# stein7/nerf-navigation

Measured on AMD Instinct MI355X. Metric: ray-samples/sec, Stonehenge-class 800x800 novel-view render, higher is better.
Workload: dtype f16

## Files before the change

nerf-navigation_amd/csrc/render_fused.hip:

```cpp
#include <atomic>
#include "ngp_mlp.h"
#include "ngp_sh.h"
#include "ngp_field.h"
#include "ngp_march.h"
#include "ngp_camera.h"

__global__ void k_field_forward_lds(rf_params P, const float* __restrict__ xyzs, const float* __restrict__ dirs, uint32_t M,
                                    float* __restrict__ sigmas, void* __restrict__ rgbs, bool rgb_half);

static int rf_field_forward(const ngp_field_t* field_host, const float* xyzs, const float* dirs, uint32_t M, float* sigmas, void* rgbs, bool rgb_half, void* stream) {
    rf_params P;
    int rc = rf_fill_params("field_forward", field_host, P);
    if (rc != NGP_OK) return rc;
    if (M == 0) return NGP_OK;
    NGP_REQUIRE(xyzs && dirs && sigmas && rgbs, "field_forward: null pointer");
    const uint32_t npairs = (M + 31) >> 5;
    uint32_t blocks = ngp_div_up(npairs, RF_BLOCK / 64);
    if (blocks > 256 * RF_FIELD_WG_PER_CU) blocks = 256 * RF_FIELD_WG_PER_CU;
    hipLaunchKernelGGL(k_field_forward_lds, dim3(blocks), dim3(RF_BLOCK), 36 * 1024, (hipStream_t)stream, P, xyzs, dirs, M, sigmas, rgbs, rgb_half);
    NGP_CHECK_LAUNCH("field_forward");
    return NGP_OK;
}

extern "C" int ngp_field_forward(const ngp_field_t* field_host, const float* xyzs, const float* dirs, uint32_t M,
                                 float* sigmas, float* rgbs, void* stream) {
    return rf_field_forward(field_host, xyzs, dirs, M, sigmas, rgbs, false, stream);
}

extern "C" int ngp_field_forward_half(const ngp_field_t* field_host, const float* xyzs, const float* dirs, uint32_t M,
                                      float* sigmas, void* rgbs_half, void* stream) {
    return rf_field_forward(field_host, xyzs, dirs, M, sigmas, rgbs_half, true, stream);
}


#ifndef RV_S
#define RV_S 12
#endif
static_assert(RV_S >= 2, "RV_S must be at least 2: the one-sample-per-round frame kernel has been removed");
#ifndef RV_BANDS
#define RV_BANDS 32u
#endif
#ifndef RV_REFILL_MIN
#define RV_REFILL_MIN 64
#endif
#ifndef RV_SLAB_STEPS
#define RV_SLAB_STEPS 16
#endif
#ifndef RV_BLOCK_THREADS
#define RV_BLOCK_THREADS 512
#endif
#ifndef RV_BLOCKS_PER_CU
#define RV_BLOCKS_PER_CU 1
#endif
static constexpr uint32_t RV_BLOCK = RV_BLOCK_THREADS;
static constexpr int RV_WAVES_PER_SIMD = (RV_BLOCK_THREADS / 256) * RV_BLOCKS_PER_CU;
static constexpr int RV_WAVES = RV_BLOCK / 64;
static constexpr uint32_t RV_LDS_W = RV_NFRAG * 1024;
static constexpr uint32_t RV_LDS_SH = RV_WAVES * 64 * 32;
static constexpr uint32_t RV_LDS_LV = 4 * 96;

struct rf_frame {
    const float* rays_o; const float* rays_d; uint32_t N;
    ngp_camera cam;
    const ngp_camera* cams; uint32_t frame_rays;
    float aabb[6]; float min_near;
    const uint8_t* bitfield; uint32_t C, H;
    float dt_gamma; uint32_t max_steps;
    float bg[3];
    float* image; float* depth; float* weights_sum;
    uint32_t* stats; uint32_t* queue;
#ifdef RV_COUNTERS
    uint32_t* hist;
#endif
    const uint32_t* coarse;
    uint32_t coarse_words;
    uint32_t tile_w;
    uint32_t skip;
    const uint32_t* occ_ext;
    float occ_unit, occ_top;
    const uint32_t* tile_perm;
};

__global__ __launch_bounds__(256) void k_build_coarse(const uint8_t* __restrict__ bitfield, uint32_t n_blocks_total,
                                                      uint32_t* __restrict__ coarse, uint32_t blocks_per_level, uint32_t C, uint32_t* __restrict__ ext) {
    const uint32_t w = blockIdx.x * 256 + threadIdx.x;
    if (w * 32 >= n_blocks_total) return;
    const uint64_t* b64 = reinterpret_cast<const uint64_t*>(bitfield);
    uint32_t bits = 0;
    #pragma unroll 8
    for (uint32_t i = 0; i < 32; i++) {
        const uint32_t blk = w * 32 + i;
        if (blk < n_blocks_total && b64[blk] != 0ull) bits |= 1u << i;
    }
    coarse[w] = bits;
    if (ext && bits) {
        uint32_t nb = 1;
        while (nb * nb * nb < blocks_per_level) nb <<= 1;
        uint32_t lo[3] = {0xFFFFFFFFu, 0xFFFFFFFFu, 0xFFFFFFFFu}, hi[3] = {0u, 0u, 0u};
        const uint32_t words_per_level = blocks_per_level / 32u, level = w / words_per_level;
        ngp_occ_extent_word(bits, w - level * words_per_level, level, C, nb, lo, hi);
        #pragma unroll
        for (int k = 0; k < 3; k++) { atomicMax(ext + k, (1u << 20) - lo[k]); atomicMax(ext + 3 + k, hi[k]); }
    }
}

struct rv_ray { float ox, oy, oz, dx, dy, dz, rdx, rdy, rdz; };
struct rv_consts {
    float bound, rbound, dt_gamma, dt_min, dt_max, rH, H3, Hf, Cf, Hm1;
    const uint8_t* grid;
    __device__ __forceinline__ int mip(int e) const { return (int)fminf(Cf - 1.0f, fmaxf(0.0f, (float)e)); }
};
__device__ __forceinline__ float rv_uniform(float v) {
    return __builtin_bit_cast(float, __builtin_amdgcn_readfirstlane(__builtin_bit_cast(int, v)));
}
struct rv_view : rv_ray, rv_consts {
    __device__ __forceinline__ rv_view(const rv_ray& r, const rv_consts& k) : rv_ray(r), rv_consts(k) {}
};

typedef ngp_point<rv_view> rv_point;

struct rv_block_cache { uint32_t blk = 0xffffffffu, lo = 0, hi = 0; };

struct rv_tested { rv_point r; bool maybe; uint32_t sw; };

__device__ __forceinline__ bool rv_test(const rv_view& m, const uint32_t* __restrict__ lds_coarse, uint32_t coarse_words, rv_block_cache& bc,
                                        float tc, rv_tested& st
#ifdef RV_COUNTERS
                                        , int* rv_dbg_ptr
#endif
                                        ) {
    rv_point& r = st.r;
    r.at(m, tc);
    const uint32_t mort = ngp_morton3((uint32_t)r.nx, (uint32_t)r.ny, (uint32_t)r.nz);
    st.maybe = true;
    st.sw = 0;
    if (lds_coarse) {
        const uint32_t blk = mort >> 6;
        st.maybe = (lds_coarse[(uint32_t)r.level * coarse_words + (blk >> 5)] >> (blk & 31u)) & 1u;
        st.sw = (uint32_t)r.level * coarse_words + ((blk >> 6) << 1);
#ifdef RV_COUNTERS
        *rv_dbg_ptr = st.maybe ? 0 : ((lds_coarse[st.sw] | lds_coarse[st.sw + 1]) == 0u ? 2 : 1);
#endif
    }
    if (!st.maybe) return false;
    if (lds_coarse) {
        const uint32_t gblk = (uint32_t)r.level * (coarse_words << 5) + (mort >> 6);
        if (gblk != bc.blk) {
            const uint2 w = reinterpret_cast<const uint2*>(m.grid)[gblk];
            bc.blk = gblk; bc.lo = w.x; bc.hi = w.y;
        }
        return (((mort & 32u) ? bc.hi : bc.lo) >> (mort & 31u)) & 1u;
    }
    const uint32_t index = (uint32_t)((float)r.level * m.H3 + (float)mort);
    return (m.grid[index >> 3] >> (index & 7u)) & 1u;
}

__device__ __forceinline__ float rv_leave(const rv_view& m, const uint32_t* __restrict__ lds_coarse, float M, const rv_tested& st, float tc) {
    const rv_point& r = st.r;
    const float tt = r.cell_exit(m, tc);
    if (lds_coarse && !st.maybe) {
        const int sh = ((lds_coarse[st.sw] | lds_coarse[st.sw + 1]) == 0u) ? 4 : 2;
        const float ta = ngp_try_skip(m, r, tc, tt, sh, M);
        if (ta >= 0.0f) return ta;
    }
    float tp;
    return ngp_advance(m, tc, tt, tp);
}

__device__ __forceinline__ bool rv_probe(const rv_ray& ray, const rv_consts& k, const uint32_t* __restrict__ lds_coarse, uint32_t coarse_words,
                                         float M, rv_block_cache& bc, float& t, float& x, float& y, float& z, float& dt
#ifdef RV_COUNTERS
                                         , int* rv_dbg_ptr
#endif
                                         ) {
    const rv_view m(ray, k);
    rv_tested st;
#ifdef RV_COUNTERS
    const bool occ = rv_test(m, lds_coarse, coarse_words, bc, t, st, rv_dbg_ptr);
#else
    const bool occ = rv_test(m, lds_coarse, coarse_words, bc, t, st);
#endif
    x = st.r.x; y = st.r.y; z = st.r.z; dt = st.r.dt;
    if (occ) return true;
    t = rv_leave(m, lds_coarse, M, st, t);
    return false;
}


template <bool FIXED>
__device__ __forceinline__ void rf_points_loop(const rf_params& P, const rf_iter_class cls_rt, const rf_lane_levels& lv, const ngp_h8* __restrict__ lds_w,
                                               const float* __restrict__ xyzs, const float* __restrict__ dirs, uint32_t M,
                                               float* __restrict__ sigmas, void* __restrict__ rgbs_v, bool rgb_half) {
    const rf_iter_class cls = FIXED ? rf_iter_class{1u, 12u, 2u} : cls_rt;
    const int lane = threadIdx.x & 63, g = lane >> 4, s = lane & 15;
    const uint32_t wave = (blockIdx.x * RF_BLOCK + threadIdx.x) >> 6, nwaves = gridDim.x * (RF_BLOCK / 64);
    const uint32_t npairs = (M + 31) >> 5;
    for (uint32_t pair = wave; pair < npairs; pair += nwaves) {
        ngp_h8 x[2];
        ngp_h4 shq[2];
        uint32_t m[2];
        #pragma unroll
        for (int n = 0; n < 2; n++) {
            m[n] = pair * 32 + 16 * n + s;
            const uint64_t mm = m[n] < M ? m[n] : 0;
            const float px = xyzs[3 * mm], py = xyzs[3 * mm + 1], pz = xyzs[3 * mm + 2];
            float sh[16];
            sh_eval<4>(dirs[3 * mm], dirs[3 * mm + 1], dirs[3 * mm + 2], P.shn, sh);
            #pragma unroll
            for (int j = 0; j < 4; j++) {
                float v = sh[j];
                if (g == 1) v = sh[4 + j];
                if (g == 2) v = sh[8 + j];
                if (g == 3) v = sh[12 + j];
                shq[n][j] = ngp_f2h(v);
            }
            x[n] = rf_encode<false>(P, lv, cls, px, py, pz);
        }
        float sg[2], cr[2], cg[2], cb[2];
        rv_mlp_tiles<2>(lds_w, lane, x, shq, sg, cr, cg, cb);
        #pragma unroll
        for (int n = 0; n < 2; n++)
            if (g == 0 && m[n] < M) {
                rv_activate(P, sg[n], cr[n], cg[n], cb[n]);
                sigmas[m[n]] = sg[n];
                if (rgb_half) {
                    _Float16* rgbs = static_cast<_Float16*>(rgbs_v);
                    rgbs[3ull * m[n]] = (_Float16)cr[n]; rgbs[3ull * m[n] + 1] = (_Float16)cg[n]; rgbs[3ull * m[n] + 2] = (_Float16)cb[n];
                } else {
                    float* rgbs = static_cast<float*>(rgbs_v);
                    rgbs[3ull * m[n]] = cr[n]; rgbs[3ull * m[n] + 1] = cg[n]; rgbs[3ull * m[n] + 2] = cb[n];
                }
            }
    }
}

__global__ __launch_bounds__(RF_BLOCK, RF_FIELD_WG_PER_CU) void k_field_forward_lds(rf_params P, const float* __restrict__ xyzs, const float* __restrict__ dirs,
                                                                    uint32_t M, float* __restrict__ sigmas, void* __restrict__ rgbs, bool rgb_half) {
    extern __shared__ __attribute__((aligned(16))) unsigned char rf_smem[];
    ngp_h8* lds_w = reinterpret_cast<ngp_h8*>(rf_smem);
    const int lane = threadIdx.x & 63, g = lane >> 4, wave = threadIdx.x >> 6;
    rv_stage_weights(P, lds_w, wave, RF_BLOCK / 64, lane);
    rf_lane_levels lv;
    rf_setup_levels(P, g, lv);
    __syncthreads();
    const rf_iter_class cls = rf_classify(lv);
    if (cls.dense == 1u && cls.select == 2u && cls.hashed == 12u) rf_points_loop<true>(P, cls, lv, lds_w, xyzs, dirs, M, sigmas, rgbs, rgb_half);
    else rf_points_loop<false>(P, cls, lv, lds_w, xyzs, dirs, M, sigmas, rgbs, rgb_half);
}

__device__ __forceinline__ void rv_ray_od(const rf_frame& F, uint32_t ray, float o[3], float d[3]) {
    if (F.rays_o) {
        #pragma unroll
        for (int k = 0; k < 3; k++) { o[k] = F.rays_o[3ull * ray + k]; d[k] = F.rays_d[3ull * ray + k]; }
    } else if (F.cams) {
        const uint32_t f = ray / F.frame_rays;
        const ngp_camera c = F.cams[f];
        o[0] = c.t[0]; o[1] = c.t[1]; o[2] = c.t[2];
        ngp_camera_ray(c, ray - f * F.frame_rays, d);
    } else {
        o[0] = F.cam.t[0]; o[1] = F.cam.t[1]; o[2] = F.cam.t[2];
        ngp_camera_ray(F.cam, ray, d);
    }
}

__device__ __forceinline__ uint32_t rv_ray_of(uint32_t idx, uint32_t tile_w) {
    if (tile_w == 0) return idx;
    const uint32_t tile = idx >> 6, in = idx & 63u, tiles_x = tile_w >> 3;
    const uint32_t ty = tile / tiles_x, tx = tile - ty * tiles_x;
    const uint32_t p = in >> 4, s = in & 15u;
    const uint32_t px = (p & 1u) * 4 + (s & 3u), py = (p >> 1) * 4 + (s >> 2);
    return (ty * 8 + py) * tile_w + tx * 8 + px;
}

static constexpr uint32_t RV_LDS_SMP = RV_WAVES * 64 * RV_S * 16;

template <bool FIXED>
__device__ __forceinline__ void rv_frame_loop(const rf_params& P, const rf_frame& F, const rf_iter_class cls_rt,
                                              const ngp_h8* __restrict__ lds_w, _Float16* lds_sh, const rf_lane_levels* lds_lv,
                                              float4* lds_smp, const uint32_t* lds_coarse, const float* lds_occ) {
    const rf_iter_class cls = FIXED ? rf_iter_class{1u, 12u, 2u} : cls_rt;
    const int lane = threadIdx.x & 63, g = lane >> 4, s = lane & 15, wave = threadIdx.x >> 6;
    const int wave_s = __builtin_amdgcn_readfirstlane(wave);

    _Float16* my_sh = lds_sh + (wave * 64 + lane) * 16;
    const _Float16* wave_sh = lds_sh + wave * 64 * 16;
    float4* my_smp = lds_smp + (wave * 64 + lane) * RV_S;
    float4* wave_smp = lds_smp + wave * 64 * RV_S;

    rv_consts K;
    K.bound = P.bound; K.rbound = rv_uniform(1.0f / P.bound); K.dt_gamma = F.dt_gamma;
    K.Hf = rv_uniform((float)F.H); K.Cf = rv_uniform((float)F.C); K.Hm1 = rv_uniform((float)(F.H - 1));
    K.rH = rv_uniform(1.0f / K.Hf);
    K.H3 = rv_uniform((float)(F.H * F.H * F.H));
    K.dt_min = rv_uniform((2.0f * 1.7320508075688772f) / (float)F.max_steps);
    K.dt_max = rv_uniform(((2.0f * 1.7320508075688772f) * (float)(1 << (F.C - 1))) / K.Hf);
    K.grid = F.bitfield;

    bool active = false;
    uint32_t ray = 0, nsamp = 0;
    rv_ray m;
    float t = 0, last_t = 0, near = 0, far = 0;
    float ws = 0, dacc = 0, cr = 0, cg = 0, cb = 0, tcomp = 0;
    bool exhausted = false;
    uint32_t rv_q = blockIdx.x & 7u, rv_q_seen = 0;
    rv_block_cache bc;
    uint32_t n_samples_local = 0, n_tiles = 0, n_capped_local = 0, n_hit_local = 0;
#ifdef RV_COUNTERS
    uint32_t n_rounds = 0, n_trips = 0, n_probe[4] = {0, 0, 0, 0};
    unsigned long long c_refill = 0, c_march = 0, c_tiles = 0, c_comp = 0;
    const unsigned long long c_start = __builtin_readcyclecounter();
    unsigned long long c_last = c_start;
#define RV_TICK(acc) { const unsigned long long c_now = __builtin_readcyclecounter(); acc += c_now - c_last; c_last = c_now; }
    uint32_t* rv_hist = F.hist;
    unsigned long long rv_t0 = 0;
    if (rv_hist) {
        unsigned long long* p0 = reinterpret_cast<unsigned long long*>(F.queue + 24);
        const unsigned long long now = wall_clock64();
        const unsigned long long old = atomicCAS(p0, 0ull, now);
        rv_t0 = __shfl(old ? old : now, 0, 64);
    }
#else
#define RV_TICK(acc)
#endif

    for (;;) {
        if (!exhausted) {
            const unsigned long long need = __ballot(!active);
            if (need && (uint32_t)__popcll(need) >= RV_REFILL_MIN) {
                const uint32_t cnt = (uint32_t)__popcll(need);
                uint32_t base = 0;
                const uint32_t n_tiles64 = (F.N + 63u) >> 6;
                const uint32_t q_lo = (uint32_t)(((unsigned long long)n_tiles64 * rv_q) / RV_BANDS) << 6;
                uint32_t q_hi = (uint32_t)(((unsigned long long)n_tiles64 * (rv_q + 1u)) / RV_BANDS) << 6;
                q_hi = q_hi < F.N ? q_hi : F.N;
                if (lane == 0) base = atomicAdd(F.queue + 32 + rv_q, cnt);
                base = __shfl(base, 0, 64) + q_lo;
                if (!active) {
                    const uint32_t idx = base + (uint32_t)__popcll(need & ((1ull << lane) - 1ull));
                    if (idx < q_hi) {
                        ray = rv_ray_of(F.tile_perm ? (F.tile_perm[idx >> 6] << 6) | (idx & 63u) : idx, F.tile_w);
                        float o[3], d[3];
                        rv_ray_od(F, ray, o, d);
                        ngp_near_far_inline(o, d, F.aabb, F.min_near, near, far);
                        if (lds_occ) {
                            float n2, f2;
                            ngp_near_far_inline(o, d, lds_occ, 0.0f, n2, f2);
                            far = f2 == 3.402823466e+38f ? near : fminf(far, f2 + lds_occ[6]);
                        }
                        m.ox = o[0]; m.oy = o[1]; m.oz = o[2];
                        m.dx = d[0]; m.dy = d[1]; m.dz = d[2];
                        m.rdx = 1.0f / m.dx; m.rdy = 1.0f / m.dy; m.rdz = 1.0f / m.dz;
                        t = near; last_t = near; tcomp = near;
                        ws = 0; dacc = 0; cr = 0; cg = 0; cb = 0; nsamp = 0;
                        float sh[16];
                        sh_eval<4>(m.dx, m.dy, m.dz, P.shn, sh);
                        #pragma unroll
                        for (int j = 0; j < 16; j++) my_sh[j] = ngp_f2h(sh[j]);
                        active = true;
                    }
                }
                if (base + cnt >= q_hi) {
                    rv_q += 8u;
                    if (rv_q >= RV_BANDS) rv_q = (rv_q + 1u) & 7u;
                    if (++rv_q_seen == RV_BANDS) exhausted = true;
                }
            }
        }
        if (__ballot(active) == 0ull) {
            if (exhausted) break;
            continue;
        }
        RV_TICK(c_refill)

        int cnt = 0;
        bool ended = false;
#ifdef RV_COUNTERS
        n_rounds++;
        const unsigned long long rv_live = __ballot(active);
#endif
        {
            rv_ray mr = m;
            float far_r = far;
            asm("" : "+v"(mr.ox), "+v"(mr.oy), "+v"(mr.oz), "+v"(mr.dx), "+v"(mr.dy), "+v"(mr.dz),
                     "+v"(mr.rdx), "+v"(mr.rdy), "+v"(mr.rdz), "+v"(far_r));
            rv_consts Kr = K;
            asm("" : "+v"(Kr.Hf), "+v"(Kr.Hm1), "+v"(Kr.Cf), "+v"(Kr.rH), "+v"(Kr.dt_min), "+v"(Kr.dt_max), "+v"(Kr.rbound), "+v"(Kr.H3));
            const float M = (active && F.skip) ? ngp_skip_margin(mr, K.bound, lds_occ ? far_r + 4.0f * K.bound : far_r) : __builtin_inff();
            const uint32_t slot0 = ((uint32_t)wave_s * 64u + __builtin_amdgcn_mbcnt_hi(~0u, __builtin_amdgcn_mbcnt_lo(~0u, 0u))) * RV_S;
            float4* const smp_w = lds_smp + slot0;
            int probes = 0;
            float t_lim = __builtin_inff();
            auto march = [&](int upto) {
                for (;;) {
#ifdef RV_COUNTERS
                    n_trips = __builtin_amdgcn_readfirstlane(n_trips) + 1;
#endif
                    if (!(t < far_r && nsamp < F.max_steps)) { ended = true; break; }
                    if (RV_SLAB_STEPS > 0 && !(t < t_lim)) break;
                    float x, y, z, dt;
#ifdef RV_COUNTERS
                    int pc = 0;
                    const bool hit = rv_probe(mr, Kr, lds_coarse, F.coarse_words, M, bc, t, x, y, z, dt, &pc);
                    n_probe[pc]++;
                    if (hit) {
#else
                    if (rv_probe(mr, Kr, lds_coarse, F.coarse_words, M, bc, t, x, y, z, dt)) {
#endif
                        smp_w[cnt] = make_float4(x, y, z, t);
                        t += dt;
                        nsamp++;
                        if (++cnt >= upto) break;
                    }
                    if (++probes >= RF_PROBES_PER_ROUND) break;
                }
            };
            if (RV_SLAB_STEPS > 0) {
                if (active) march(1);
                const float t_first = cnt ? smp_w[0].w : __builtin_inff();
                float tf = t_first;
                #pragma unroll
                for (int off = 1; off < 64; off <<= 1) tf = fminf(tf, __shfl_xor(tf, off, 64));
                t_lim = tf + (float)RV_SLAB_STEPS * K.dt_min;
                if (cnt && !(t_first < t_lim)) { t = t_first; nsamp--; cnt = 0; ended = false; }
                if (active && cnt && !ended) march(RV_S);
            } else if (active) {
                march(RV_S);
            }
        }

        __builtin_amdgcn_fence(__ATOMIC_RELEASE, "wavefront");
        __builtin_amdgcn_wave_barrier();
        __builtin_amdgcn_fence(__ATOMIC_ACQUIRE, "wavefront");

        RV_TICK(c_march)
        int col_src;
        {
            uint32_t rank = 0, above = 0;
            const uint32_t below_me = __builtin_amdgcn_mbcnt_hi(~0u, __builtin_amdgcn_mbcnt_lo(~0u, 0u));
            #pragma unroll
            for (int c = RV_S; c >= 0; c--) {
                const unsigned long long mc = __ballot(cnt == c);
                if (cnt == c) rank = above + (uint32_t)__popcll(mc & ((1ull << below_me) - 1ull));
                above += (uint32_t)__popcll(mc);
            }
            col_src = __builtin_amdgcn_ds_permute((int)(rank << 2), (int)below_me);
        }
        #pragma unroll 1
        for (int p = 0; p < 4; p++) {
            const int src = __shfl(col_src, 16 * p + s, 64);
            const int ccol = __shfl(cnt, src, 64);
            if (__ballot(ccol > 0) == 0ull) continue;
            const ngp_h4 shq = *reinterpret_cast<const ngp_h4*>(wave_sh + src * 16 + 4 * g);
            const rf_lane_levels lv = lds_lv[g];
            #pragma unroll 1
            for (int k = 0; k < RV_S; k += 2) {
                if (__ballot(ccol > k) == 0ull) break;
                if (k + 1 < RV_S && __ballot(ccol > k + 1) != 0ull) {
                    ngp_h8 xs[2];
                    #pragma unroll
                    for (int n = 0; n < 2; n++) {
                        float4 q = wave_smp[src * RV_S + k + n];
                        if (!(ccol > k + n)) q = make_float4(0.f, 0.f, 0.f, 0.f);
                        xs[n] = rf_encode<true>(P, lv, cls, q.x, q.y, q.z);
                    }
                    n_tiles += 2;
                    const ngp_h4 ss[2] = {shq, shq};
                    float a[2], b[2], c[2], d[2];
                    rv_mlp_tiles<2>(lds_w, lane, xs, ss, a, b, c, d);
                    #pragma unroll
                    for (int n = 0; n < 2; n++)
                        if (g == 0 && ccol > k + n) {
                            ngp_h4 r;
                            r[0] = (_Float16)a[n]; r[1] = (_Float16)b[n]; r[2] = (_Float16)c[n]; r[3] = (_Float16)d[n];
                            *reinterpret_cast<ngp_h4*>(&wave_smp[src * RV_S + k + n]) = r;
                        }
                } else {
                    float4 q = wave_smp[src * RV_S + k];
                    if (!(ccol > k)) q = make_float4(0.f, 0.f, 0.f, 0.f);
                    n_tiles++;
                    float a, b, c, d;
                    rv_field_tile(P, lv, cls, lds_w, lane, q.x, q.y, q.z, shq, a, b, c, d);
                    if (g == 0 && ccol > k) {
                        ngp_h4 r;
                        r[0] = (_Float16)a; r[1] = (_Float16)b; r[2] = (_Float16)c; r[3] = (_Float16)d;
                        *reinterpret_cast<ngp_h4*>(&wave_smp[src * RV_S + k]) = r;
                    }
                }
            }
        }

        __builtin_amdgcn_fence(__ATOMIC_RELEASE, "wavefront");
        __builtin_amdgcn_wave_barrier();
        __builtin_amdgcn_fence(__ATOMIC_ACQUIRE, "wavefront");

        RV_TICK(c_tiles)
        bool done = false;
        for (int k = 0; k < cnt; k++) {
            const ngp_h4 r = *reinterpret_cast<const ngp_h4*>(&my_smp[k]);
            const float ts = my_smp[k].w;
            const float dt = ngp_clampf(ts * K.dt_gamma, K.dt_min, K.dt_max);
            const float ta = ts + dt;
            const float d1 = ta - last_t;
            last_t = ta;
            float sig = (float)r[0], sr = (float)r[1], sg = (float)r[2], sb = (float)r[3];
            rv_activate(P, sig, sr, sg, sb);
            n_samples_local++;
            const float alpha = 1.0f - ngp_expf(-sig * dt);
            const float T = 1 - ws;
            const float w = alpha * T;
            ws += w;
            tcomp += d1;
            dacc += w * tcomp;
            cr += w * sr; cg += w * sg; cb += w * sb;
            if ((double)T < 1e-4) {
                done = true;
#ifdef RV_COUNTERS
                n_probe[3] += (uint32_t)(cnt - (k + 1));
#endif
                break;
            }
        }
        float far0 = far;
        if (lds_occ && (done || ended)) {
            const float o3[3] = {m.ox, m.oy, m.oz}, d3[3] = {m.dx, m.dy, m.dz};
            float n0;
            ngp_near_far_inline(o3, d3, F.aabb, F.min_near, n0, far0);
        }
        const bool capped = !done && ended && nsamp >= F.max_steps && t < far0;
        if (ended) done = true;
        if (done) {
            F.image[3ull * ray] = cr + (1 - ws) * F.bg[0];
            F.image[3ull * ray + 1] = cg + (1 - ws) * F.bg[1];
            F.image[3ull * ray + 2] = cb + (1 - ws) * F.bg[2];
            F.depth[ray] = fmaxf(dacc - near, 0.0f) / (far0 - near);
            F.weights_sum[ray] = ws;
            n_capped_local += capped ? 1u : 0u;
            n_hit_local += nsamp > 0 ? 1u : 0u;
            active = false;
        }
        RV_TICK(c_comp)
#ifdef RV_COUNTERS
        if (rv_hist) {
            const unsigned long long now = wall_clock64();
            const uint32_t bin = now > rv_t0 ? (uint32_t)((now - rv_t0) / 2000ull) : 0u;
            uint32_t rs = (uint32_t)cnt;
            #pragma unroll
            for (int off = 32; off > 0; off >>= 1) rs += __shfl_down(rs, off, 64);
            if (lane == 0 && bin < 512u) {
                atomicAdd(rv_hist + bin, rs); atomicAdd(rv_hist + 512 + bin, 1u);
                atomicAdd(rv_hist + 1024 + bin, (uint32_t)__popcll(rv_live));
            }
        }
#endif
    }
#ifdef RV_COUNTERS
    if (rv_hist && lane == 0) {
        const unsigned long long now = wall_clock64();
        const uint32_t bin = now > rv_t0 ? (uint32_t)((now - rv_t0) / 2000ull) : 0u;
        if (bin < 512u) atomicAdd(rv_hist + 1536 + bin, 1u);
    }
#endif
    uint32_t tot = n_samples_local, tot_capped = n_capped_local, tot_hit = n_hit_local;
    #pragma unroll
    for (int off = 32; off > 0; off >>= 1) {
        tot += __shfl_down(tot, off, 64);
        tot_capped += __shfl_down(tot_capped, off, 64);
        tot_hit += __shfl_down(tot_hit, off, 64);
    }
    if (lane == 0 && tot) atomicAdd(F.stats, tot);
    if (lane == 0 && tot_capped) atomicAdd(F.stats + 1, tot_capped);
    if (lane == 0 && tot_hit) atomicAdd(F.stats + 2, tot_hit);
    if (lane == 0 && n_tiles) atomicAdd(F.stats + 3, n_tiles);
#ifdef RV_COUNTERS
    if (lane == 0) { atomicAdd(F.queue + 1, n_rounds); atomicAdd(F.queue + 2, n_trips); }
    atomicAdd(F.queue + 3, n_probe[0]); atomicAdd(F.queue + 4, n_probe[1]); atomicAdd(F.queue + 5, n_probe[2]); atomicAdd(F.queue + 6, n_probe[3]);
    if (lane == 0) {
        unsigned long long* c = reinterpret_cast<unsigned long long*>(F.queue + 8);
        const unsigned long long c_total = __builtin_readcyclecounter() - c_start;
        atomicAdd(c + 0, c_refill); atomicAdd(c + 1, c_march); atomicAdd(c + 2, c_tiles); atomicAdd(c + 3, c_comp);
        atomicAdd(c + 4, c_total); atomicMax(c + 5, c_total); atomicMax(c + 6, ~c_total);
    }
#endif
}

__global__ __launch_bounds__(RV_BLOCK, RV_WAVES_PER_SIMD) void k_render_frame_multi(rf_params P, rf_frame F) {
    extern __shared__ __attribute__((aligned(16))) unsigned char rv_smem[];
    ngp_h8* lds_w = reinterpret_cast<ngp_h8*>(rv_smem);
    _Float16* lds_sh = reinterpret_cast<_Float16*>(rv_smem + RV_LDS_W);
    rf_lane_levels* lds_lv = reinterpret_cast<rf_lane_levels*>(rv_smem + RV_LDS_W + RV_LDS_SH);
    float4* lds_smp = reinterpret_cast<float4*>(rv_smem + RV_LDS_W + RV_LDS_SH + RV_LDS_LV);
    uint32_t* lds_coarse = F.coarse ? reinterpret_cast<uint32_t*>(rv_smem + RV_LDS_W + RV_LDS_SH + RV_LDS_LV + RV_LDS_SMP) : nullptr;

    const int lane = threadIdx.x & 63, g = lane >> 4, s = lane & 15, wave = threadIdx.x >> 6;

    rv_stage_weights(P, lds_w, wave, RV_WAVES, lane);
    if (lds_coarse) {
        const uint32_t nw = F.coarse_words * F.C;
        for (uint32_t i = threadIdx.x; i < nw; i += RV_BLOCK) lds_coarse[i] = F.coarse[i];
    }
    float* lds_occ = (lds_coarse && F.occ_ext) ? reinterpret_cast<float*>(lds_coarse + F.coarse_words * F.C) : nullptr;
    if (lds_occ && threadIdx.x < 3) {
        const uint32_t k = threadIdx.x;
        const uint32_t hi = F.occ_ext[3 + k], lo = (1u << 20) - F.occ_ext[k];
        const bool any = F.occ_ext[3] != 0u;
        lds_occ[k] = any ? -F.occ_top + ((float)lo - 1.0f) * F.occ_unit : 3.0e38f;
        lds_occ[3 + k] = any ? -F.occ_top + ((float)hi + 1.0f) * F.occ_unit : 3.1e38f;
        if (k == 0) lds_occ[6] = 2.0f * (((2.0f * 1.7320508075688772f) * (float)(1 << (F.C - 1))) / (float)F.H);
    }
    if (wave == 0 && s == 0) {
        rf_lane_levels tmp;
        rf_setup_levels(P, g, tmp);
        lds_lv[g] = tmp;
    }
    __syncthreads();
    const rf_iter_class cls = rf_classify(lds_lv[g]);
    if (cls.dense == 1u && cls.select == 2u && cls.hashed == 12u)
        rv_frame_loop<true>(P, F, cls, lds_w, lds_sh, lds_lv, lds_smp, lds_coarse, lds_occ);
    else
        rv_frame_loop<false>(P, F, cls, lds_w, lds_sh, lds_lv, lds_smp, lds_coarse, lds_occ);
}

static constexpr uint32_t RV_ORDER_MAX = 4096;

__global__ __launch_bounds__(256) void k_tile_cost(rf_frame F, float bound, uint32_t n_tiles, uint32_t* __restrict__ cost) {
    const uint32_t tile = blockIdx.x * 4u + (threadIdx.x >> 6), lane = threadIdx.x & 63u;
    if (tile >= n_tiles) return;
    rv_consts K;
    K.bound = bound; K.rbound = 1.0f / bound; K.dt_gamma = F.dt_gamma;
    K.Hf = (float)F.H; K.Cf = (float)F.C; K.Hm1 = (float)(F.H - 1); K.rH = 1.0f / K.Hf; K.H3 = (float)(F.H * F.H * F.H);
    K.dt_min = (2.0f * 1.7320508075688772f) / (float)F.max_steps;
    K.dt_max = ((2.0f * 1.7320508075688772f) * (float)(1 << (F.C - 1))) / K.Hf;
    K.grid = F.bitfield;
    float box[7] = {0.f, 0.f, 0.f, 0.f, 0.f, 0.f, 0.f};
    if (F.occ_ext) {
        const bool any = F.occ_ext[3] != 0u;
        #pragma unroll
        for (int k = 0; k < 3; k++) {
            const uint32_t hi = F.occ_ext[3 + k], lo = (1u << 20) - F.occ_ext[k];
            box[k] = any ? -F.occ_top + ((float)lo - 1.0f) * F.occ_unit : 3.0e38f;
            box[3 + k] = any ? -F.occ_top + ((float)hi + 1.0f) * F.occ_unit : 3.1e38f;
        }
        box[6] = 2.0f * K.dt_max;
    }
    const uint32_t tiles_x = F.tile_w >> 3, ty = tile / tiles_x, tx = tile - ty * tiles_x;
    float acc = 0.0f;
    #pragma unroll
    for (int r = 0; r < 5; r++) {
        const uint32_t px = r == 4 ? 4u : (r & 1) * 7u, py = r == 4 ? 4u : (r >> 1) * 7u;
        float o[3], d[3], near, far;
        rv_ray_od(F, (ty * 8u + py) * F.tile_w + tx * 8u + px, o, d);
        ngp_near_far_inline(o, d, F.aabb, F.min_near, near, far);
        if (F.occ_ext) {
            float n2, f2;
            ngp_near_far_inline(o, d, box, 0.0f, n2, f2);
            far = f2 == 3.402823466e+38f ? near : fminf(far, f2 + box[6]);
        }
        rv_ray m;
        m.ox = o[0]; m.oy = o[1]; m.oz = o[2]; m.dx = d[0]; m.dy = d[1]; m.dz = d[2]; m.rdx = m.rdy = m.rdz = 0.0f;
        const rv_view v(m, K);
        const float seg = far > near ? (far - near) * (1.0f / 64.0f) : 0.0f;
        rv_point pt;
        pt.at(v, (far > near ? near : 0.0f) + ((float)lane + 0.5f) * seg);
        const uint32_t blk = ngp_morton3((uint32_t)pt.nx, (uint32_t)pt.ny, (uint32_t)pt.nz) >> 6;
        if ((F.coarse[(uint32_t)pt.level * F.coarse_words + (blk >> 5)] >> (blk & 31u)) & 1u) acc += seg / pt.dt;
    }
    #pragma unroll
    for (int off = 32; off > 0; off >>= 1) acc += __shfl_xor(acc, off, 64);
    if (lane == 0) cost[tile] = (uint32_t)fminf(acc + 0.5f, 4.0e9f);
}

__global__ __launch_bounds__(1024) void k_tile_sort(const uint32_t* __restrict__ cost, uint32_t n_tiles, uint32_t* __restrict__ perm) {
    __shared__ __attribute__((aligned(16))) uint32_t c[RV_ORDER_MAX];
    const uint32_t b = blockIdx.x;
    const uint32_t lo = (uint32_t)(((unsigned long long)n_tiles * b) / RV_BANDS), hi = (uint32_t)(((unsigned long long)n_tiles * (b + 1u)) / RV_BANDS);
    const uint32_t n = hi - lo, n4 = (n + 3u) & ~3u;
    for (uint32_t i = threadIdx.x; i < n4; i += 1024u) c[i] = i < n ? cost[lo + i] : 0u;
    __syncthreads();
    const uint4* c4 = reinterpret_cast<const uint4*>(c);
    for (uint32_t i = threadIdx.x; i < n; i += 1024u) {
        const uint32_t ci = c[i];
        uint32_t rank = 0;
        #pragma unroll 4
        for (uint32_t j = 0; j < n4; j += 4u) {
            const uint4 q = c4[j >> 2];
            rank += (q.x > ci || (q.x == ci && j < i)) ? 1u : 0u;
            rank += (q.y > ci || (q.y == ci && j + 1u < i)) ? 1u : 0u;
            rank += (q.z > ci || (q.z == ci && j + 2u < i)) ? 1u : 0u;
            rank += (q.w > ci || (q.w == ci && j + 3u < i)) ? 1u : 0u;
        }
        perm[lo + rank] = lo + i;
    }
}

static inline bool rv_pow2(uint32_t v) { return v && !(v & (v - 1)); }

static std::atomic<int> rv_occ_box_enabled{1};
extern "C" int ngp_render_set_occupied_box(int enabled) { return rv_occ_box_enabled.exchange(enabled ? 1 : 0, std::memory_order_relaxed); }
static std::atomic<int> rv_block_skip_enabled{1};
extern "C" int ngp_render_set_block_skip(int enabled) { return rv_block_skip_enabled.exchange(enabled ? 1 : 0, std::memory_order_relaxed); }
static std::atomic<int> rv_tile_order_enabled{1};
extern "C" int ngp_render_set_tile_order(int enabled) { return rv_tile_order_enabled.exchange(enabled ? 1 : 0, std::memory_order_relaxed); }

static constexpr size_t RV_WS_COARSE = 256, RV_WS_HIST = RV_WS_COARSE + 36 * 1024, RV_WS_AREA = 256 + 48 * 1024;
static_assert(RV_LDS_W + RV_LDS_SH + RV_LDS_LV + RV_LDS_SMP + 36 * 1024 > 160 * 1024, "the coarse map could reach RV_WS_HIST");
static_assert(RV_WS_HIST + 2048 * sizeof(uint32_t) <= RV_WS_AREA, "workspace carve");
extern "C" size_t ngp_render_frame_workspace(uint32_t N) {
    return RV_WS_AREA + 2 * sizeof(uint32_t) * (size_t)ngp_div_up(N, 64u);
}

static int rv_fill_camera(const char* who, const float* pose_host, const float* intrinsics_host, uint32_t H, uint32_t W, ngp_camera& cam) {
    NGP_REQUIRE(pose_host && intrinsics_host, "camera: pose / intrinsics are host pointers and must not be null");
    NGP_REQUIRE(H >= 1 && W >= 1 && (uint64_t)H * W <= 0xFFFFFFFFull, "camera: bad image size");
    NGP_REQUIRE(intrinsics_host[0] != 0.0f && intrinsics_host[1] != 0.0f, "camera: zero focal length");
    for (int r = 0; r < 3; r++) {
        for (int c = 0; c < 3; c++) cam.r[3 * r + c] = pose_host[4 * r + c];
        cam.t[r] = pose_host[4 * r + 3];
    }
    cam.fx = intrinsics_host[0]; cam.fy = intrinsics_host[1]; cam.cx = intrinsics_host[2]; cam.cy = intrinsics_host[3];
    cam.W = W; cam.H = H;
    (void)who;
    return NGP_OK;
}

static int rv_render_frame(const ngp_field_t* field_host, const float* rays_o, const float* rays_d, const ngp_camera* cam, uint32_t n_cams, uint32_t N,
                           uint32_t image_width, const float* aabb_host, float min_near, const uint8_t* bitfield, uint32_t C, uint32_t Hgrid,
                           float dt_gamma, uint32_t max_steps, const float* bg_color3_host,
                           float* image, float* depth, float* weights_sum, uint32_t* stats,
                           void* workspace, size_t workspace_bytes, void* stream) {
    rf_params P;
    int rc = rf_fill_params("render_frame", field_host, P);
    if (rc != NGP_OK) return rc;
    NGP_REQUIRE(stats && workspace && workspace_bytes >= RV_WS_COARSE, "render_frame: stats / workspace missing");
    NGP_REQUIRE(aabb_host && bg_color3_host, "render_frame: aabb / bg_color are host pointers and must not be null");
    NGP_REQUIRE(C >= 1 && C <= 16 && Hgrid >= 1 && Hgrid <= 1024 && max_steps >= 1, "render_frame: bad C/H/max_steps");
    NGP_REQUIRE(rv_pow2(Hgrid), "render_frame: the grid size must be a power of two (cells are addressed by Morton index)");
    hipStream_t s = (hipStream_t)stream;
    if (hipMemsetAsync(stats, 0, 4 * sizeof(uint32_t), s) != hipSuccess || hipMemsetAsync(workspace, 0, RV_WS_COARSE, s) != hipSuccess)
        return ngp_fail(NGP_ELAUNCH, "render_frame: memset failed");
    if (N == 0) return NGP_OK;
    NGP_REQUIRE((cam || (rays_o && rays_d)) && bitfield && image && depth && weights_sum, "render_frame: null pointer");
    rf_frame F;
    F.rays_o = cam ? nullptr : rays_o; F.rays_d = cam ? nullptr : rays_d; F.N = N;
    F.cam = cam ? *cam : ngp_camera{};
    F.cams = nullptr; F.frame_rays = N;
    if (cam && n_cams > 1) {
        const size_t at = (ngp_render_frame_workspace(N) + 255) & ~(size_t)255;
        NGP_REQUIRE(workspace_bytes >= at + n_cams * sizeof(ngp_camera), "render_frames_camera: workspace too small (ngp_render_frames_workspace)");
        ngp_camera* dst = reinterpret_cast<ngp_camera*>(reinterpret_cast<unsigned char*>(workspace) + at);
        if (hipMemcpyAsync(dst, cam, n_cams * sizeof(ngp_camera), hipMemcpyHostToDevice, s) != hipSuccess) return ngp_fail(NGP_ELAUNCH, "render_frames_camera: camera copy failed");
        F.cams = dst; F.frame_rays = N / n_cams;
    }
    for (int i = 0; i < 6; i++) F.aabb[i] = aabb_host[i];
    F.min_near = min_near; F.bitfield = bitfield; F.C = C; F.H = Hgrid;
    F.dt_gamma = dt_gamma; F.max_steps = max_steps;
    for (int i = 0; i < 3; i++) F.bg[i] = bg_color3_host[i];
    F.image = image; F.depth = depth; F.weights_sum = weights_sum;
    F.stats = stats; F.queue = (uint32_t*)workspace;
#ifdef RV_COUNTERS
    F.hist = nullptr;
#ifdef RV_TIMELINE
    if (workspace_bytes >= RV_WS_HIST + 2048 * sizeof(uint32_t)) {
        F.hist = reinterpret_cast<uint32_t*>(reinterpret_cast<unsigned char*>(workspace) + RV_WS_HIST);
        if (hipMemsetAsync(F.hist, 0, 2048 * sizeof(uint32_t), s) != hipSuccess) return ngp_fail(NGP_ELAUNCH, "render_frame: memset failed");
    }
#endif
#endif
    F.tile_w = 0;
    const uint32_t hint = image_width;
    if (hint >= 8 && hint % 8 == 0 && N % hint == 0 && (N / hint) % 8 == 0) F.tile_w = hint;

    F.coarse = nullptr; F.coarse_words = 0; F.skip = 0; F.occ_ext = nullptr; F.occ_unit = 0.0f; F.occ_top = 0.0f;
    F.tile_perm = nullptr;
    static_assert(sizeof(rf_lane_levels) * 4 == RV_LDS_LV, "LDS carve of the level table");
    size_t lds = RV_LDS_W + RV_LDS_SH + RV_LDS_LV + RV_LDS_SMP;
    const void* kernel = reinterpret_cast<const void*>(k_render_frame_multi);
    const uint64_t blocks_per_level = (uint64_t)Hgrid * Hgrid * Hgrid / 64;
    const uint64_t coarse_bytes = (uint64_t)C * blocks_per_level / 8;
    if (rv_pow2(Hgrid) && Hgrid >= 8 && blocks_per_level % 32 == 0 && lds + coarse_bytes <= 160 * 1024 && (uint64_t)C * Hgrid * Hgrid * Hgrid <= (1ull << 24) &&
        workspace_bytes >= RV_WS_COARSE + coarse_bytes && (reinterpret_cast<uintptr_t>(bitfield) & 7u) == 0) {
        uint32_t* coarse = reinterpret_cast<uint32_t*>(reinterpret_cast<unsigned char*>(workspace) + RV_WS_COARSE);
        const uint32_t n_blocks_total = (uint32_t)(C * blocks_per_level);
        F.coarse = coarse;
        F.coarse_words = (uint32_t)(blocks_per_level / 32);
        lds += coarse_bytes;
        uint32_t* ext = nullptr;
        int e2;
        const bool nested = Hgrid >= 64 && (C == 1 || frexpf(field_host->bound, &e2) == 0.5f);
        if (nested && rv_occ_box_enabled.load(std::memory_order_relaxed) && lds + 32 <= 160 * 1024) {
            ext = reinterpret_cast<uint32_t*>(workspace) + 26;
            F.occ_ext = ext;
            F.occ_top = C == 1 ? field_host->bound : (float)(1u << (C - 1));
            F.occ_unit = 2.0f * (C == 1 ? field_host->bound : 1.0f) / (float)(Hgrid / 4);
            lds += 32;
        }
        hipLaunchKernelGGL(k_build_coarse, dim3(ngp_div_up(n_blocks_total / 32, 256)), dim3(256), 0, s, bitfield, n_blocks_total, coarse,
                           (uint32_t)blocks_per_level, C, ext);
        int e;
        F.skip = (rv_block_skip_enabled.load(std::memory_order_relaxed) && Hgrid >= 64 && (C == 1 || frexpf(field_host->bound, &e) == 0.5f)) ? 1u : 0u;
    }
    const uint32_t n_tiles = F.tile_w ? N / 64u : 0u;
    if (n_tiles && !F.cams && F.coarse && rv_tile_order_enabled.load(std::memory_order_relaxed) && ngp_div_up(n_tiles, RV_BANDS) <= RV_ORDER_MAX &&
        workspace_bytes >= RV_WS_AREA + 2 * sizeof(uint32_t) * (size_t)n_tiles) {
        uint32_t* perm = reinterpret_cast<uint32_t*>(reinterpret_cast<unsigned char*>(workspace) + RV_WS_AREA);
        uint32_t* cost = perm + n_tiles;
        hipLaunchKernelGGL(k_tile_cost, dim3(ngp_div_up(n_tiles, 4u)), dim3(256), 0, s, F, P.bound, n_tiles, cost);
        hipLaunchKernelGGL(k_tile_sort, dim3(RV_BANDS), dim3(1024), 0, s, cost, n_tiles, perm);
        NGP_CHECK_LAUNCH("render_frame: tile order");
        F.tile_perm = perm;
    }
    NGP_REQUIRE(lds <= 160 * 1024, "render_frame: LDS carve exceeds 160 KiB");
    static std::atomic<unsigned long long> attr_devices{0};
    int device = 0;
    if (hipGetDevice(&device) != hipSuccess || device < 0) return ngp_fail(NGP_ELAUNCH, "render_frame: no current device");
    const unsigned long long device_bit = 1ull << (device & 63);
    if (device >= 64 || !(attr_devices.load(std::memory_order_acquire) & device_bit)) {
        if (hipFuncSetAttribute(kernel, hipFuncAttributeMaxDynamicSharedMemorySize, 160 * 1024) != hipSuccess)
            return ngp_fail(NGP_ELAUNCH, "render_frame: cannot raise the dynamic LDS limit");
        attr_devices.fetch_or(device_bit, std::memory_order_release);
    }
    uint32_t blocks = 256 * RV_BLOCKS_PER_CU;
    const uint32_t need = ngp_div_up(N, RV_BLOCK);
    if (blocks > need) blocks = need;
    hipLaunchKernelGGL(k_render_frame_multi, dim3(blocks), dim3(RV_BLOCK), lds, s, P, F);
    NGP_CHECK_LAUNCH("render_frame");
    return NGP_OK;
}

extern "C" int ngp_render_frame(const ngp_field_t* field_host, const float* rays_o, const float* rays_d, uint32_t N,
                                uint32_t image_width, const float* aabb_host, float min_near, const uint8_t* bitfield, uint32_t C, uint32_t Hgrid,
                                float dt_gamma, uint32_t max_steps, const float* bg_color3_host,
                                float* image, float* depth, float* weights_sum, uint32_t* stats,
                                void* workspace, size_t workspace_bytes, void* stream) {
    return rv_render_frame(field_host, rays_o, rays_d, nullptr, 0, N, image_width, aabb_host, min_near, bitfield, C, Hgrid, dt_gamma, max_steps,
                           bg_color3_host, image, depth, weights_sum, stats, workspace, workspace_bytes, stream);
}

extern "C" int ngp_render_frame_camera(const ngp_field_t* field_host, const float* pose_host, const float* intrinsics_host, uint32_t H, uint32_t W,
                                       const float* aabb_host, float min_near, const uint8_t* bitfield, uint32_t C, uint32_t Hgrid,
                                       float dt_gamma, uint32_t max_steps, const float* bg_color3_host,
                                       float* image, float* depth, float* weights_sum, uint32_t* stats,
                                       void* workspace, size_t workspace_bytes, void* stream) {
    ngp_camera cam;
    const int rc = rv_fill_camera("render_frame_camera", pose_host, intrinsics_host, H, W, cam);
    if (rc != NGP_OK) return rc;
    return rv_render_frame(field_host, nullptr, nullptr, &cam, 1, H * W, W, aabb_host, min_near, bitfield, C, Hgrid, dt_gamma, max_steps,
                           bg_color3_host, image, depth, weights_sum, stats, workspace, workspace_bytes, stream);
}

extern "C" size_t ngp_render_frames_workspace(uint32_t P, uint32_t rays_per_frame) {
    return ((ngp_render_frame_workspace(P * rays_per_frame) + 255) & ~(size_t)255) + (size_t)P * sizeof(ngp_camera);
}

extern "C" int ngp_render_frames_camera(const ngp_field_t* field_host, const float* poses_host, uint32_t P, const float* intrinsics_host, uint32_t H, uint32_t W,
                                        const float* aabb_host, float min_near, const uint8_t* bitfield, uint32_t C, uint32_t Hgrid,
                                        float dt_gamma, uint32_t max_steps, const float* bg_color3_host,
                                        float* image, float* depth, float* weights_sum, uint32_t* stats,
                                        void* workspace, size_t workspace_bytes, void* stream) {
    NGP_REQUIRE(P >= 1 && P <= 64, "render_frames_camera: 1..64 frames per launch");
    NGP_REQUIRE(H % 8 == 0 && W % 8 == 0, "render_frames_camera: H and W must be multiples of 8");
    NGP_REQUIRE((uint64_t)P * H * W <= 0xFFFFFFFFull, "render_frames_camera: too many rays");
    NGP_REQUIRE(poses_host, "render_frames_camera: poses is a host pointer and must not be null");
    ngp_camera cams[64];
    for (uint32_t p = 0; p < P; p++) {
        const int rc = rv_fill_camera("render_frames_camera", poses_host + 16 * p, intrinsics_host, H, W, cams[p]);
        if (rc != NGP_OK) return rc;
    }
    return rv_render_frame(field_host, nullptr, nullptr, cams, P, P * H * W, W, aabb_host, min_near, bitfield, C, Hgrid, dt_gamma, max_steps,
                           bg_color3_host, image, depth, weights_sum, stats, workspace, workspace_bytes, stream);
}

__global__ __launch_bounds__(256) void k_get_rays(ngp_camera cam, const int64_t* __restrict__ inds, uint32_t N,
                                                  float* __restrict__ rays_o, float* __restrict__ rays_d) {
    const uint32_t k = blockIdx.x * 256 + threadIdx.x;
    if (k >= N) return;
    uint32_t pixel = k;
    if (inds) {
        const int64_t p = inds[k];
        const int64_t last = (int64_t)cam.W * cam.H - 1;
        pixel = (uint32_t)(p < 0 ? 0 : p > last ? last : p);
    }
    float d[3];
    ngp_camera_ray(cam, pixel, d);
    #pragma unroll
    for (int c = 0; c < 3; c++) { rays_o[3ull * k + c] = cam.t[c]; rays_d[3ull * k + c] = d[c]; }
}

extern "C" int ngp_get_rays(const float* pose_host, const float* intrinsics_host, uint32_t H, uint32_t W,
                            const int64_t* inds, uint32_t N, float* rays_o, float* rays_d, void* stream) {
    ngp_camera cam;
    const int rc = rv_fill_camera("get_rays", pose_host, intrinsics_host, H, W, cam);
    if (rc != NGP_OK) return rc;
    if (N == 0) return NGP_OK;
    NGP_REQUIRE(inds || (uint64_t)N == (uint64_t)H * W, "get_rays: N must be H * W when inds is null");
    NGP_REQUIRE(rays_o && rays_d, "get_rays: null pointer");
    hipLaunchKernelGGL(k_get_rays, dim3(ngp_div_up(N, 256u)), dim3(256), 0, (hipStream_t)stream, cam, inds, N, rays_o, rays_d);
    NGP_CHECK_LAUNCH("get_rays");
    return NGP_OK;
}
```

Baseline: 9.500 billion.

## Fold stats clear into coarse build, wave-reduce extent atomics, batch tile-cost loads

Several unrelated tweaks. The coarse-map kernel now zeroes the stats counters, which removes one memset launch, and it reduces the occupancy-extent maxima across each wave with shuffles so only one lane issues the atomics. The tile-cost kernel gathers its five coarse-word loads before testing them, and the per-group MLP evaluation moves into a helper with the tile width pinned to a scalar register. It also adds debug wall-clock counters under RV_COUNTERS, and stats clearing now depends on which launch path runs, which makes the ordering assumptions more fragile.

After: 9.479 billion. Within noise of the previous version (-0.2%).

```diff
diff --git a/nerf-navigation_amd/csrc/render_fused.hip b/nerf-navigation_amd/csrc/render_fused.hip
--- a/nerf-navigation_amd/csrc/render_fused.hip
+++ b/nerf-navigation_amd/csrc/render_fused.hip
@@ -71,6 +71,7 @@
     uint32_t* stats; uint32_t* queue;
 #ifdef RV_COUNTERS
     uint32_t* hist;
+    uint32_t* dbg;
 #endif
     const uint32_t* coarse;
     uint32_t coarse_words;
@@ -82,25 +83,45 @@
 };
 
 __global__ __launch_bounds__(256) void k_build_coarse(const uint8_t* __restrict__ bitfield, uint32_t n_blocks_total,
-                                                      uint32_t* __restrict__ coarse, uint32_t blocks_per_level, uint32_t C, uint32_t* __restrict__ ext) {
+                                                      uint32_t* __restrict__ coarse, uint32_t blocks_per_level, uint32_t C, uint32_t* __restrict__ ext,
+                                                      uint32_t* __restrict__ stats) {
+    if (blockIdx.x == 0 && threadIdx.x < 4u) stats[threadIdx.x] = 0u;
     const uint32_t w = blockIdx.x * 256 + threadIdx.x;
-    if (w * 32 >= n_blocks_total) return;
+    const bool in = w * 32 < n_blocks_total;
     const uint64_t* b64 = reinterpret_cast<const uint64_t*>(bitfield);
     uint32_t bits = 0;
-    #pragma unroll 8
-    for (uint32_t i = 0; i < 32; i++) {
-        const uint32_t blk = w * 32 + i;
-        if (blk < n_blocks_total && b64[blk] != 0ull) bits |= 1u << i;
-    }
-    coarse[w] = bits;
-    if (ext && bits) {
-        uint32_t nb = 1;
-        while (nb * nb * nb < blocks_per_level) nb <<= 1;
-        uint32_t lo[3] = {0xFFFFFFFFu, 0xFFFFFFFFu, 0xFFFFFFFFu}, hi[3] = {0u, 0u, 0u};
-        const uint32_t words_per_level = blocks_per_level / 32u, level = w / words_per_level;
-        ngp_occ_extent_word(bits, w - level * words_per_level, level, C, nb, lo, hi);
+    if (in) {
+        #pragma unroll 8
+        for (uint32_t i = 0; i < 32; i++) {
+            const uint32_t blk = w * 32 + i;
+            if (blk < n_blocks_total && b64[blk] != 0ull) bits |= 1u << i;
+        }
+        coarse[w] = bits;
+    }
+    if (ext) {
+        uint32_t v[6] = {0u, 0u, 0u, 0u, 0u, 0u};
+        if (bits) {
+            uint32_t nb = 1;
+            while (nb * nb * nb < blocks_per_level) nb <<= 1;
+            uint32_t lo[3] = {0xFFFFFFFFu, 0xFFFFFFFFu, 0xFFFFFFFFu}, hi[3] = {0u, 0u, 0u};
+            const uint32_t words_per_level = blocks_per_level / 32u, level = w / words_per_level;
+            ngp_occ_extent_word(bits, w - level * words_per_level, level, C, nb, lo, hi);
+            #pragma unroll
+            for (int k = 0; k < 3; k++) { v[k] = (1u << 20) - lo[k]; v[3 + k] = hi[k]; }
+        }
         #pragma unroll
-        for (int k = 0; k < 3; k++) { atomicMax(ext + k, (1u << 20) - lo[k]); atomicMax(ext + 3 + k, hi[k]); }
+        for (int k = 0; k < 6; k++) {
+            #pragma unroll
+            for (int off = 1; off < 64; off <<= 1) {
+                const uint32_t other = (uint32_t)__shfl_xor((int)v[k], off, 64);
+                v[k] = v[k] > other ? v[k] : other;
+            }
+        }
+        if ((threadIdx.x & 63u) == 0u) {
+            #pragma unroll
+            for (int k = 0; k < 6; k++)
+                if (v[k]) atomicMax(ext + k, v[k]);
+        }
     }
 }
 
@@ -274,18 +295,61 @@
 
 static constexpr uint32_t RV_LDS_SMP = RV_WAVES * 64 * RV_S * 16;
 
+__device__ __forceinline__ uint32_t rv_eval_group(const rf_params& P, const rf_iter_class cls, const ngp_h8* __restrict__ lds_w, const rf_lane_levels* lds_lv,
+                                                  const _Float16* wave_sh, float4* wave_smp, int lane, int src, int ccol) {
+    const int g = lane >> 4;
+    uint32_t n_tiles = 0;
+    if (__ballot(ccol > 0) == 0ull) return 0u;
+    const ngp_h4 shq = *reinterpret_cast<const ngp_h4*>(wave_sh + src * 16 + 4 * g);
+    const rf_lane_levels lv = lds_lv[g];
+    #pragma unroll 1
+    for (int k = 0; k < RV_S; k += 2) {
+        if (__ballot(ccol > k) == 0ull) break;
+        if (k + 1 < RV_S && __ballot(ccol > k + 1) != 0ull) {
+            ngp_h8 xs[2];
+            #pragma unroll
+            for (int n = 0; n < 2; n++) {
+                float4 q = wave_smp[src * RV_S + k + n];
+                if (!(ccol > k + n)) q = make_float4(0.f, 0.f, 0.f, 0.f);
+                xs[n] = rf_encode<true>(P, lv, cls, q.x, q.y, q.z);
+            }
+            n_tiles += 2;
+            const ngp_h4 ss[2] = {shq, shq};
+            float a[2], b[2], c[2], d[2];
+            rv_mlp_tiles<2>(lds_w, lane, xs, ss, a, b, c, d);
+            #pragma unroll
+            for (int n = 0; n < 2; n++)
+                if (g == 0 && ccol > k + n) {
+                    ngp_h4 r;
+                    r[0] = (_Float16)a[n]; r[1] = (_Float16)b[n]; r[2] = (_Float16)c[n]; r[3] = (_Float16)d[n];
+                    *reinterpret_cast<ngp_h4*>(&wave_smp[src * RV_S + k + n]) = r;
+                }
+        } else {
+            float4 q = wave_smp[src * RV_S + k];
+            if (!(ccol > k)) q = make_float4(0.f, 0.f, 0.f, 0.f);
+            n_tiles++;
+            float a, b, c, d;
+            rv_field_tile(P, lv, cls, lds_w, lane, q.x, q.y, q.z, shq, a, b, c, d);
+            if (g == 0 && ccol > k) {
+                ngp_h4 r;
+                r[0] = (_Float16)a; r[1] = (_Float16)b; r[2] = (_Float16)c; r[3] = (_Float16)d;
+                *reinterpret_cast<ngp_h4*>(&wave_smp[src * RV_S + k]) = r;
+            }
+        }
+    }
+    return n_tiles;
+}
+
 template <bool FIXED>
 __device__ __forceinline__ void rv_frame_loop(const rf_params& P, const rf_frame& F, const rf_iter_class cls_rt,
                                               const ngp_h8* __restrict__ lds_w, _Float16* lds_sh, const rf_lane_levels* lds_lv,
                                               float4* lds_smp, const uint32_t* lds_coarse, const float* lds_occ) {
     const rf_iter_class cls = FIXED ? rf_iter_class{1u, 12u, 2u} : cls_rt;
-    const int lane = threadIdx.x & 63, g = lane >> 4, s = lane & 15, wave = threadIdx.x >> 6;
+    const int lane = threadIdx.x & 63, s = lane & 15, wave = threadIdx.x >> 6;
     const int wave_s = __builtin_amdgcn_readfirstlane(wave);
 
     _Float16* my_sh = lds_sh + (wave * 64 + lane) * 16;
-    const _Float16* wave_sh = lds_sh + wave * 64 * 16;
     float4* my_smp = lds_smp + (wave * 64 + lane) * RV_S;
-    float4* wave_smp = lds_smp + wave * 64 * RV_S;
 
     rv_consts K;
     K.bound = P.bound; K.rbound = rv_uniform(1.0f / P.bound); K.dt_gamma = F.dt_gamma;
@@ -313,10 +377,11 @@
 #define RV_TICK(acc) { const unsigned long long c_now = __builtin_readcyclecounter(); acc += c_now - c_last; c_last = c_now; }
     uint32_t* rv_hist = F.hist;
     unsigned long long rv_t0 = 0;
-    if (rv_hist) {
+    if (rv_hist || F.dbg) {
         unsigned long long* p0 = reinterpret_cast<unsigned long long*>(F.queue + 24);
         const unsigned long long now = wall_clock64();
-        const unsigned long long old = atomicCAS(p0, 0ull, now);
+        unsigned long long old = 0;
+        if (lane == 0) old = atomicCAS(p0, 0ull, now);
         rv_t0 = __shfl(old ? old : now, 0, 64);
     }
 #else
@@ -338,7 +403,9 @@
                 if (!active) {
                     const uint32_t idx = base + (uint32_t)__popcll(need & ((1ull << lane) - 1ull));
                     if (idx < q_hi) {
-                        ray = rv_ray_of(F.tile_perm ? (F.tile_perm[idx >> 6] << 6) | (idx & 63u) : idx, F.tile_w);
+                        uint32_t tile_w = F.tile_w;
+                        asm volatile("" : "+s"(tile_w));
+                        ray = rv_ray_of(F.tile_perm ? (F.tile_perm[idx >> 6] << 6) | (idx & 63u) : idx, tile_w);
                         float o[3], d[3];
                         rv_ray_od(F, ray, o, d);
                         ngp_near_far_inline(o, d, F.aabb, F.min_near, near, far);
@@ -367,8 +434,16 @@
             }
         }
         if (__ballot(active) == 0ull) {
-            if (exhausted) break;
-            continue;
+            if (!exhausted) continue;
+#ifdef RV_COUNTERS
+            if (F.dbg && lane == 0) {
+                const unsigned long long now = wall_clock64() - rv_t0;
+                unsigned long long* d64 = reinterpret_cast<unsigned long long*>(F.dbg);
+                atomicAdd(d64 + 0, now); atomicMax(d64 + 2, now); atomicAdd(d64 + 5, 1ull);
+                if (atomicAdd(F.dbg + 64 + blockIdx.x, 1u) == (uint32_t)RV_WAVES - 1u) { atomicAdd(d64 + 1, now); atomicAdd(d64 + 6, 1ull); }
+            }
+#endif
+            break;
         }
         RV_TICK(c_refill)
 
@@ -449,44 +524,7 @@
         for (int p = 0; p < 4; p++) {
             const int src = __shfl(col_src, 16 * p + s, 64);
             const int ccol = __shfl(cnt, src, 64);
-            if (__ballot(ccol > 0) == 0ull) continue;
-            const ngp_h4 shq = *reinterpret_cast<const ngp_h4*>(wave_sh + src * 16 + 4 * g);
-            const rf_lane_levels lv = lds_lv[g];
-            #pragma unroll 1
-            for (int k = 0; k < RV_S; k += 2) {
-                if (__ballot(ccol > k) == 0ull) break;
-                if (k + 1 < RV_S && __ballot(ccol > k + 1) != 0ull) {
-                    ngp_h8 xs[2];
-                    #pragma unroll
-                    for (int n = 0; n < 2; n++) {
-                        float4 q = wave_smp[src * RV_S + k + n];
-                        if (!(ccol > k + n)) q = make_float4(0.f, 0.f, 0.f, 0.f);
-                        xs[n] = rf_encode<true>(P, lv, cls, q.x, q.y, q.z);
-                    }
-                    n_tiles += 2;
-                    const ngp_h4 ss[2] = {shq, shq};
-                    float a[2], b[2], c[2], d[2];
-                    rv_mlp_tiles<2>(lds_w, lane, xs, ss, a, b, c, d);
-                    #pragma unroll
-                    for (int n = 0; n < 2; n++)
-                        if (g == 0 && ccol > k + n) {
-                            ngp_h4 r;
-                            r[0] = (_Float16)a[n]; r[1] = (_Float16)b[n]; r[2] = (_Float16)c[n]; r[3] = (_Float16)d[n];
-                            *reinterpret_cast<ngp_h4*>(&wave_smp[src * RV_S + k + n]) = r;
-                        }
-                } else {
-                    float4 q = wave_smp[src * RV_S + k];
-                    if (!(ccol > k)) q = make_float4(0.f, 0.f, 0.f, 0.f);
-                    n_tiles++;
-                    float a, b, c, d;
-                    rv_field_tile(P, lv, cls, lds_w, lane, q.x, q.y, q.z, shq, a, b, c, d);
-                    if (g == 0 && ccol > k) {
-                        ngp_h4 r;
-                        r[0] = (_Float16)a; r[1] = (_Float16)b; r[2] = (_Float16)c; r[3] = (_Float16)d;
-                        *reinterpret_cast<ngp_h4*>(&wave_smp[src * RV_S + k]) = r;
-                    }
-                }
-            }
+            n_tiles += rv_eval_group(P, cls, lds_w, lds_lv, lds_sh + wave_s * 64 * 16, lds_smp + wave_s * 64 * RV_S, lane, src, ccol);
         }
 
         __builtin_amdgcn_fence(__ATOMIC_RELEASE, "wavefront");
@@ -643,7 +681,8 @@
         box[6] = 2.0f * K.dt_max;
     }
     const uint32_t tiles_x = F.tile_w >> 3, ty = tile / tiles_x, tx = tile - ty * tiles_x;
-    float acc = 0.0f;
+    uint32_t word[5], bit[5];
+    float steps[5];
     #pragma unroll
     for (int r = 0; r < 5; r++) {
         const uint32_t px = r == 4 ? 4u : (r & 1) * 7u, py = r == 4 ? 4u : (r >> 1) * 7u;
@@ -662,8 +701,17 @@
         rv_point pt;
         pt.at(v, (far > near ? near : 0.0f) + ((float)lane + 0.5f) * seg);
         const uint32_t blk = ngp_morton3((uint32_t)pt.nx, (uint32_t)pt.ny, (uint32_t)pt.nz) >> 6;
-        if ((F.coarse[(uint32_t)pt.level * F.coarse_words + (blk >> 5)] >> (blk & 31u)) & 1u) acc += seg / pt.dt;
-    }
+        word[r] = (uint32_t)pt.level * F.coarse_words + (blk >> 5);
+        bit[r] = blk & 31u;
+        steps[r] = seg / pt.dt;
+    }
+    uint32_t w[5];
+    #pragma unroll
+    for (int r = 0; r < 5; r++) w[r] = F.coarse[word[r]];
+    float acc = 0.0f;
+    #pragma unroll
+    for (int r = 0; r < 5; r++)
+        if ((w[r] >> bit[r]) & 1u) acc += steps[r];
     #pragma unroll
     for (int off = 32; off > 0; off >>= 1) acc += __shfl_xor(acc, off, 64);
     if (lane == 0) cost[tile] = (uint32_t)fminf(acc + 0.5f, 4.0e9f);
@@ -702,6 +750,8 @@
 extern "C" int ngp_render_set_tile_order(int enabled) { return rv_tile_order_enabled.exchange(enabled ? 1 : 0, std::memory_order_relaxed); }
 
 static constexpr size_t RV_WS_COARSE = 256, RV_WS_HIST = RV_WS_COARSE + 36 * 1024, RV_WS_AREA = 256 + 48 * 1024;
+static constexpr size_t RV_WS_DBG = RV_WS_HIST + 2048 * sizeof(uint32_t) + 256, RV_WS_DBG_BYTES = (64 + 256 * RV_BLOCKS_PER_CU) * sizeof(uint32_t);
+static_assert(RV_WS_DBG + RV_WS_DBG_BYTES <= RV_WS_AREA, "workspace carve");
 static_assert(RV_LDS_W + RV_LDS_SH + RV_LDS_LV + RV_LDS_SMP + 36 * 1024 > 160 * 1024, "the coarse map could reach RV_WS_HIST");
 static_assert(RV_WS_HIST + 2048 * sizeof(uint32_t) <= RV_WS_AREA, "workspace carve");
 extern "C" size_t ngp_render_frame_workspace(uint32_t N) {
@@ -735,9 +785,12 @@
     NGP_REQUIRE(C >= 1 && C <= 16 && Hgrid >= 1 && Hgrid <= 1024 && max_steps >= 1, "render_frame: bad C/H/max_steps");
     NGP_REQUIRE(rv_pow2(Hgrid), "render_frame: the grid size must be a power of two (cells are addressed by Morton index)");
     hipStream_t s = (hipStream_t)stream;
-    if (hipMemsetAsync(stats, 0, 4 * sizeof(uint32_t), s) != hipSuccess || hipMemsetAsync(workspace, 0, RV_WS_COARSE, s) != hipSuccess)
-        return ngp_fail(NGP_ELAUNCH, "render_frame: memset failed");
-    if (N == 0) return NGP_OK;
+    if (hipMemsetAsync(workspace, 0, RV_WS_COARSE, s) != hipSuccess) return ngp_fail(NGP_ELAUNCH, "render_frame: memset failed");
+    bool stats_cleared = false;
+    if (N == 0) {
+        if (hipMemsetAsync(stats, 0, 4 * sizeof(uint32_t), s) != hipSuccess) return ngp_fail(NGP_ELAUNCH, "render_frame: memset failed");
+        return NGP_OK;
+    }
     NGP_REQUIRE((cam || (rays_o && rays_d)) && bitfield && image && depth && weights_sum, "render_frame: null pointer");
     rf_frame F;
     F.rays_o = cam ? nullptr : rays_o; F.rays_d = cam ? nullptr : rays_d; F.N = N;
@@ -757,7 +810,11 @@
     F.image = image; F.depth = depth; F.weights_sum = weights_sum;
     F.stats = stats; F.queue = (uint32_t*)workspace;
 #ifdef RV_COUNTERS
-    F.hist = nullptr;
+    F.hist = nullptr; F.dbg = nullptr;
+    if (workspace_bytes >= RV_WS_AREA) {
+        F.dbg = reinterpret_cast<uint32_t*>(reinterpret_cast<unsigned char*>(workspace) + RV_WS_DBG);
+        if (hipMemsetAsync(F.dbg, 0, RV_WS_DBG_BYTES, s) != hipSuccess) return ngp_fail(NGP_ELAUNCH, "render_frame: memset failed");
+    }
 #ifdef RV_TIMELINE
     if (workspace_bytes >= RV_WS_HIST + 2048 * sizeof(uint32_t)) {
         F.hist = reinterpret_cast<uint32_t*>(reinterpret_cast<unsigned char*>(workspace) + RV_WS_HIST);
@@ -794,10 +851,12 @@
             lds += 32;
         }
         hipLaunchKernelGGL(k_build_coarse, dim3(ngp_div_up(n_blocks_total / 32, 256)), dim3(256), 0, s, bitfield, n_blocks_total, coarse,
-                           (uint32_t)blocks_per_level, C, ext);
+                           (uint32_t)blocks_per_level, C, ext, stats);
+        stats_cleared = true;
         int e;
         F.skip = (rv_block_skip_enabled.load(std::memory_order_relaxed) && Hgrid >= 64 && (C == 1 || frexpf(field_host->bound, &e) == 0.5f)) ? 1u : 0u;
     }
+    if (!stats_cleared && hipMemsetAsync(stats, 0, 4 * sizeof(uint32_t), s) != hipSuccess) return ngp_fail(NGP_ELAUNCH, "render_frame: memset failed");
     const uint32_t n_tiles = F.tile_w ? N / 64u : 0u;
     if (n_tiles && !F.cams && F.coarse && rv_tile_order_enabled.load(std::memory_order_relaxed) && ngp_div_up(n_tiles, RV_BANDS) <= RV_ORDER_MAX &&
         workspace_bytes >= RV_WS_AREA + 2 * sizeof(uint32_t) * (size_t)n_tiles) {
```
